# Madhudorai/encodec-pytorch

Hardware: AMD Instinct MI355X
Metric: audio-seconds/sec EnCodec24k train step, batch 32x1s (higher is better)
Workload: dtype f32; 1 GPU; config 3: 24 kHz mono full GAN (MS-STFT disc + Balancer); global_batch=32, parallelism=dp1

## Files before the change

### encodec-pytorch_amd/csrc/api.hip

```cpp
#include <stdarg.h>
#include <stdio.h>
#include <stdlib.h>
#include <string.h>

#include <atomic>
#include <mutex>

#include "common.h"
#include "prof.h"

namespace {
constexpr int kMaxSlots = 1 << 14;
struct ProfState {
    std::mutex mu;
    bool on = false;
    int next = 0;
    hipEvent_t ev0[kMaxSlots];
    hipEvent_t ev1[kMaxSlots];
    double flops[kMaxSlots];
    double bytes[kMaxSlots];
    bool timed[kMaxSlots];
    char tags[kMaxSlots][64];
    bool created = false;
};
ProfState g_prof;
std::atomic<bool> g_prof_on{false};

struct OptDef {
    EncxOpt id;
    const char* name;
    int64_t def;
};
constexpr OptDef kOpts[OPT_COUNT] = {
    {OPT_FFT, "FFT", 1}, {OPT_PW, "PW", 1}, {OPT_PW_TMAX, "PW_TMAX", 1024}, {OPT_PW_WG_TMAX, "PW_WG_TMAX", 12000}, {OPT_LSTM_FUSE, "LSTM_FUSE", 0},
    {OPT_LSTM_PERSIST, "LSTM_PERSIST", 1},
    {OPT_LSTM_WG_SPLITS, "LSTM_WG_SPLITS", 32},
    {OPT_FWR, "FWR", 256}, {OPT_DGR, "DGR", 256}, {OPT_WGR, "WGR", 2048},
    {OPT_WGR_WGS, "WGR_WGS", 256}, {OPT_FEAT_CODE, "FEAT_CODE", 1}, {OPT_CONV_CK, "CONV_CK", 64},
    {OPT_CONV_SPLIT, "CONV_SPLIT", 1024}, {OPT_CONV_WG_SPLIT, "CONV_WG_SPLIT", 1024},
    {OPT_CONV2, "CONV2", 7}, {OPT_CONV2_TILE, "CONV2_TILE", 0}, {OPT_CONV2_RED, "CONV2_RED", 64},
    {OPT_CONV2_KS, "CONV2_KS", 0}, {OPT_CONV2_WGS, "CONV2_WGS", 512},
    {OPT_CONV2_LOWT, "CONV2_LOWT", 0},
    {OPT_LSTM_SPIN, "LSTM_SPIN", 0}, {OPT_LSTM_FAULT, "LSTM_FAULT", 0},
    {OPT_BLAS, "BLAS", 3},
};
constexpr bool opts_in_order() {
    for (int i = 0; i < OPT_COUNT; ++i)
        if (kOpts[i].id != i) return false;
    return true;
}
static_assert(opts_in_order(), "kOpts must list every EncxOpt in enum order");
std::atomic<int64_t> g_opt[OPT_COUNT];
std::once_flag g_opt_once;
void opt_init() {
    std::call_once(g_opt_once, [] {
        for (int i = 0; i < OPT_COUNT; ++i) {
            char env[64];
            snprintf(env, sizeof(env), "ENCX_%s", kOpts[i].name);
            const char* v = getenv(env);
            g_opt[i].store(v ? atoll(v) : kOpts[i].def);
        }
    });
}
int opt_find(const char* name) {
    if (!name) return -1;
    if (!strncmp(name, "ENCX_", 5)) name += 5;
    for (int i = 0; i < OPT_COUNT; ++i)
        if (!strcmp(name, kOpts[i].name)) return i;
    return -1;
}
}

int64_t encx_opt(EncxOpt id) {
    opt_init();
    return g_opt[id].load(std::memory_order_relaxed);
}

// ... 119 lines not shown
```

### encodec-pytorch_amd/csrc/common.h

```cpp
#pragma once
#include <hip/hip_runtime.h>
#include <algorithm>
#include <stdint.h>

#include "../../include/encx.h"

#define ENCX_DEV __device__ __forceinline__

typedef float f32x16 __attribute__((ext_vector_type(16)));
typedef float f32x4 __attribute__((ext_vector_type(4)));
typedef float f32x2 __attribute__((ext_vector_type(2)));
typedef float f32x4u __attribute__((ext_vector_type(4), aligned(4)));
ENCX_DEV f32x4 ld4u(const float* p) { return *(const f32x4u*)p; }

#define ENCX_CHECK_LAUNCH()                                                    \
    do {                                                                       \
        hipError_t _e = hipGetLastError();                                     \
        if (_e != hipSuccess) return (int)_e;                                  \
    } while (0)
#define ENCX_REQUIRE(cond)                                                     \
    do {                                                                       \
        if (!(cond)) return ENCX_EINVAL;                                       \
    } while (0)

// ... 128 lines not shown
    t.x = id % gx;
    t.y = (id / gx) % gy;
    t.z = id / (gx * gy);
    return t;
}

static inline int64_t cdiv(int64_t a, int64_t b) { return (a + b - 1) / b; }

enum EncxOpt {
    OPT_FFT,
    OPT_PW,
    OPT_PW_TMAX,
    OPT_PW_WG_TMAX,
    OPT_LSTM_FUSE,
    OPT_LSTM_PERSIST,
    OPT_LSTM_WG_SPLITS,
    OPT_FWR,
    OPT_DGR,
    OPT_WGR,
    OPT_WGR_WGS,
    OPT_FEAT_CODE,
    OPT_CONV_CK,
    OPT_CONV_SPLIT,
    OPT_CONV_WG_SPLIT,
    OPT_CONV2,
    OPT_CONV2_TILE,
    OPT_CONV2_RED,
    OPT_CONV2_KS,
    OPT_CONV2_WGS,
    OPT_CONV2_LOWT,
    OPT_LSTM_SPIN,
    OPT_LSTM_FAULT,
    OPT_BLAS,
    OPT_COUNT
};
int64_t encx_opt(EncxOpt id);

int encx_sgemm(hipStream_t st, bool ta, bool tb, int m, int n, int k, const float* A, int lda, const float* B,
               int ldb, float* C, int ldc, bool accumulate, int batch = 1, int64_t sa = 0, int64_t sb = 0,
               int64_t sc = 0);
```

### encodec-pytorch_amd/csrc/gemm.h

```cpp
#pragma once
#include "common.h"

template <class EP, class = void>
struct ep_npre { static constexpr int value = 0; };
template <class EP>
struct ep_npre<EP, decltype((void)EP::NPRE)> { static constexpr int value = EP::NPRE; };

template <class LD, class = void>
struct ld_vec { static constexpr bool value = false; };
template <class LD>
struct ld_vec<LD, decltype((void)LD::VEC)> { static constexpr bool value = LD::VEC; };

template <int BM, int BN, int WM, int WN, int BK, class LD, class EP>
__global__ __launch_bounds__(256) void gemm_kernel(LD ld, EP ep, int M, int N, int Kred, int kchunk) {
    constexpr int TM = BM / WM / 32, TN = BN / WN / 32;
    __shared__ float As[BK][BM + 1];
    __shared__ float Bs[BK][BN + 1];
    const int tid = threadIdx.x, lane = tid & 63, wave = tid >> 6;
    const int wm0 = (wave / WN) * TM * 32, wn0 = (wave % WN) * TN * 32;
    const int m0 = blockIdx.y * BM, n0 = blockIdx.x * BN;
    const int kbeg = blockIdx.z * kchunk, kend = min(Kred, kbeg + kchunk);
    const int h = lane >> 5, l32 = lane & 31;
    f32x16 acc[TM][TN];
#pragma unroll
    for (int i = 0; i < TM; ++i)
#pragma unroll
        for (int j = 0; j < TN; ++j) acc[i][j] = (f32x16){0};
    constexpr int EA = BM * BK / 256, EB = BN * BK / 256;
    static_assert(EA * 256 == BM * BK && EB * 256 == BN * BK, "tile/thread mismatch");
    float ra[EA], rb[EB];
    constexpr bool VEC = ld_vec<LD>::value;
    static_assert(!VEC || (EA % 4 == 0 && EB % 4 == 0), "quad staging");
    auto quad_a = [&](int e, int& m, int& k) {
        const int i = tid + e * 256;
        if (LD::A_K_FAST) { m = i / (BK / 4); k = (i - m * (BK / 4)) * 4; }
        else { k = i / (BM / 4); m = (i - k * (BM / 4)) * 4; }
    };
    auto quad_b = [&](int e, int& k, int& n) {
        const int i = tid + e * 256;
        if (LD::B_N_FAST) { k = i / (BN / 4); n = (i - k * (BN / 4)) * 4; }
        else { n = i / (BK / 4); k = (i - n * (BK / 4)) * 4; }
    };
    auto fetch = [&](int k0) {
        if constexpr (VEC) {
#pragma unroll
            for (int e = 0; e < EA / 4; ++e) {
                int m, k;
                quad_a(e, m, k);
                const int gm = m0 + m, gk = k0 + k;
                const bool whole = LD::A_K_FAST ? (gm < M && gk + 3 < kend) : (gm + 3 < M && gk < kend);
                f32x4 v;
                if (whole) {
                    v = ld.a4(gm, gk);
                } else {
// ... 135 lines not shown
                for (int r = 0; r < 16; ++r) {
                    const int m = m0 + wm0 + i * 32 + mfma_row(r, lane);
                    if (m < M && n < N) ep(m, n, acc[i][j][r]);
                }
            }
        }
}

struct GemmShape {
    int BM, BN;
    int64_t blocks;
};

static inline GemmShape gemm_shape(int M, int N) {
    GemmShape s;
    if (N <= 48) { s.BM = 128; s.BN = 32; }
    else if (N <= 96) { s.BM = 128; s.BN = 64; }
    else if (cdiv(N, 128) * cdiv(M, 128) < 512) { s.BM = 64; s.BN = 64; }
    else { s.BM = 128; s.BN = 128; }
    s.blocks = cdiv(N, s.BN) * cdiv(M, s.BM);
    return s;
}

static inline int gemm_splits(int M, int N, int Kred, int min_k = 256, int max_splits = 32) {
    GemmShape s = gemm_shape(M, N);
    int sp = (int)cdiv(1024, s.blocks);
    int cap = Kred / min_k;
    if (sp > cap) sp = cap;
    if (sp > max_splits) sp = max_splits;
    return sp < 1 ? 1 : sp;
}

template <class LD, class EP>
int gemm_launch(const LD& ld, const EP& ep, int M, int N, int Kred, hipStream_t st, int splits = 1) {
    GemmShape s = gemm_shape(M, N);
    const int kchunk = splits > 1 ? (int)(cdiv(cdiv(Kred, splits), 32) * 32) : Kred;
    const int z = (int)cdiv(Kred, kchunk);
    if (s.BN == 32) {
        hipLaunchKernelGGL((gemm_kernel<128, 32, 4, 1, 32, LD, EP>), dim3(cdiv(N, 32), cdiv(M, 128), z),
                           dim3(256), 0, st, ld, ep, M, N, Kred, kchunk);
    } else if (s.BN == 64 && s.BM == 128) {
        hipLaunchKernelGGL((gemm_kernel<128, 64, 2, 2, 32, LD, EP>), dim3(cdiv(N, 64), cdiv(M, 128), z),
                           dim3(256), 0, st, ld, ep, M, N, Kred, kchunk);
    } else if (s.BN == 64) {
        hipLaunchKernelGGL((gemm_kernel<64, 64, 2, 2, 32, LD, EP>), dim3(cdiv(N, 64), cdiv(M, 64), z),
                           dim3(256), 0, st, ld, ep, M, N, Kred, kchunk);
    } else {
        hipLaunchKernelGGL((gemm_kernel<128, 128, 2, 2, 32, LD, EP>), dim3(cdiv(N, 128), cdiv(M, 128), z),
                           dim3(256), 0, st, ld, ep, M, N, Kred, kchunk);
    }
    ENCX_CHECK_LAUNCH();
    return 0;
}

static inline int gemm_splits_128(int M, int N, int Kred, int min_k = 256, int max_splits = 32) {
    const int blocks = (int)(cdiv(N, 128) * cdiv(M, 128));
    int sp = (int)cdiv(1024, blocks);
    const int cap = Kred / min_k;
    if (sp > cap) sp = cap;
    if (sp > max_splits) sp = max_splits;
    return sp < 1 ? 1 : sp;
}
template <class LD, class EP>
int gemm_launch_128(const LD& ld, const EP& ep, int M, int N, int Kred, hipStream_t st, int splits) {
    const int kchunk = splits > 1 ? (int)(cdiv(cdiv(Kred, splits), 32) * 32) : Kred;
    const int z = (int)cdiv(Kred, kchunk);
    hipLaunchKernelGGL((gemm_kernel<128, 128, 2, 2, 32, LD, EP>), dim3(cdiv(N, 128), cdiv(M, 128), z),
                       dim3(256), 0, st, ld, ep, M, N, Kred, kchunk);
    ENCX_CHECK_LAUNCH();
    return 0;
// ... 8 lines not shown
```

### encodec-pytorch_amd/csrc/rvq.hip

```cpp
#include "common.h"
#include "prof.h"
#include "gemm.h"

namespace {

constexpr int NT = 256;

struct Rows {
    const float* p;
    int64_t sB, sT, sD;
    int Tf;
    FastDiv fTf;
    ENCX_DEV float at(int n, int d) const {
        const int b = (int)fdiv((uint32_t)n, fTf), t = n - b * Tf;
        return p[b * sB + t * sT + d * sD];
    }
};

ENCX_DEV uint32_t ord_key(float f) {
    uint32_t u = __float_as_uint(f);
    return (u & 0x80000000u) ? ~u : (u | 0x80000000u);
}
ENCX_DEV uint64_t umin64(uint64_t a, uint64_t b) { return a < b ? a : b; }
ENCX_DEV uint64_t shfl_xor64(uint64_t v, int o) {
// ... 94 lines not shown
        ee[c] = v;
    }
    f32x16 acc[1];
    acc[0] = (f32x16){0};
    const float* ap = As + h * AR_ROWS + wm0 + l32;
    const float* bp = Bs + h * AR_BS + wn0 + l32;
#pragma unroll 4
    for (int dp = 0; dp < D; dp += 2) {
        const float av = ap[dp * AR_ROWS];
        acc[0] = mfma32(av, bp[dp * AR_BS], acc[0]);
    }
    __syncthreads();
#pragma unroll
    for (int r = 0; r < 16; ++r) {
        const int row = wm0 + mfma_row(r, lane);
        uint64_t best = ~0ull;
#pragma unroll
        for (int j = 0; j < 1; ++j) {
            const int c = wn0 + j * 32 + l32, k = k0 + c;
            if (k < Kc) {
                const float v = (xx[row] - 2.f * acc[j][r]) + ee[c];
                best = umin64(best, ((uint64_t)ord_key(v) << 32) | (uint32_t)k);
            }
        }
#pragma unroll
        for (int o = 16; o > 0; o >>= 1) best = umin64(best, shfl_xor64(best, o));
        if (l32 == 0) part[wave & 1][row] = best;
    }
    __syncthreads();
    if (tid < AR_ROWS && n0 + tid < N)
        atomicMin((unsigned long long*)&keys[n0 + tid], (unsigned long long)umin64(part[0][tid], part[1][tid]));
}

constexpr int DR_ROWS = 32;

__global__ __launch_bounds__(NT) void rvq_argmin_direct(Rows x, const float* embed, uint64_t* keys,
                                                        int N, int D, int Kc) {
    extern __shared__ float sm[];
    float* es = sm;
    float* xs = sm + NT * (D + 1);
    __shared__ uint64_t part[4];
    const int tid = threadIdx.x, lane = tid & 63, wave = tid >> 6;
    const int n0 = blockIdx.x * DR_ROWS, k = blockIdx.y * NT + tid;
    for (int i = tid; i < NT * D; i += NT) {
        int c = i / D, d = i - c * D, kk = blockIdx.y * NT + c;
        es[c * (D + 1) + d] = kk < Kc ? embed[(int64_t)kk * D + d] : 0.f;
    }
    for (int i = tid; i < DR_ROWS * D; i += NT) {
        int r = i / D, d = i - r * D;
        xs[i] = (n0 + r < N) ? x.at(n0 + r, d) : 0.f;
    }
    __syncthreads();
    for (int r = 0; r < DR_ROWS; ++r) {
        float s = 0.f;
        for (int d = 0; d < D; ++d) {
            float df = xs[r * D + d] - es[tid * (D + 1) + d];
            s = fmaf(df, df, s);
        }
        uint64_t key = k < Kc ? (((uint64_t)ord_key(s) << 32) | (uint32_t)k) : ~0ull;
#pragma unroll
        for (int o = 32; o > 0; o >>= 1) key = umin64(key, shfl_xor64(key, o));
        if (lane == 0) part[wave] = key;
        __syncthreads();
        if (tid == 0 && n0 + r < N) {
            uint64_t b = umin64(umin64(part[0], part[1]), umin64(part[2], part[3]));
            atomicMin((unsigned long long*)&keys[n0 + r], (unsigned long long)b);
// ... 21 lines not shown
    __shared__ float red[16];
    float s = 0.f;
    for (int64_t i = (int64_t)blockIdx.x * NT + threadIdx.x; i < total; i += (int64_t)gridDim.x * NT) {
        int64_t bd = i / Tf;
        int t = (int)(i - bd * Tf);
        int64_t b = bd / D;
        int d = (int)(bd - b * D);
        const int64_t k = idx[b * Tf + t];
        const float x = xin[i];
        const float q = embed[k * D + d];
        const float qs = ste ? x + (q - x) : q;
        res[i] = x - qs;
        if (out) out[i] = first ? qs : out[i] + qs;
        if (cdir) cdir[i] = first ? (x - qs) : cdir[i] + (x - qs);
        const float df = qs - x;
        s = fmaf(df, df, s);
    }
    s = block_sum(s, red);
    if (parts && threadIdx.x == 0) parts[blockIdx.x] = s;
}

__global__ void rvq_gather_kernel(const float* embed, const int64_t* idx, float* out, int D, int Tf,
                                  int64_t total, int acc) {
    int64_t i = (int64_t)blockIdx.x * blockDim.x + threadIdx.x;
    if (i >= total) return;
    int64_t bd = i / Tf;
    int t = (int)(i - bd * Tf);
    int64_t b = bd / D;
    int d = (int)(bd - b * D);
    float q = embed[idx[b * Tf + t] * D + d];
    out[i] = acc ? out[i] + q : q;
}

struct LdOneHot {
    static constexpr bool A_K_FAST = true, B_N_FAST = false;
    Rows x;
    const int64_t* idx;
    int D;
    ENCX_DEV float a(int c, int n) const { return idx[n] == c ? 1.f : 0.f; }
    ENCX_DEV float b(int n, int d) const { return d < D ? x.at(n, d) : 1.f; }
};
struct EpSlab {
    float* ws;
    int Kc, W;
    ENCX_DEV void operator()(int c, int d, float v) const {
        ws[((int64_t)blockIdx.z * Kc + c) * W + d] = v;
    }
};

template <int MODE>
__global__ void bucket_finish(const float* ws, int S, int Kc, int D, float* cs, float* ea,
                              float* means, int64_t* bins, float decay, float one_m) {
    const int c = blockIdx.x, W = D + 1;
    const float cnt = MODE == 1 ? sum_strided(ws + (int64_t)c * W + D, S, (int64_t)Kc * W) : 0.f;
    for (int d = threadIdx.x; d <= D; d += blockDim.x) {
        const float s = sum_strided(ws + (int64_t)c * W + d, S, (int64_t)Kc * W);
        if (MODE == 2) {
            means[(int64_t)c * W + d] = s;
        } else if (MODE == 0) {
            if (d < D) {
                float* p = ea + (int64_t)c * D + d;
                *p = fmaf(s, one_m, *p * decay);
            } else {
                cs[c] = fmaf(s, one_m, cs[c] * decay);
            }
        } else {
            if (d < D) {
                if (cnt > 0.f) means[(int64_t)c * D + d] = s / cnt;
            } else {
                bins[c] = (int64_t)cnt;
            }
        }
    }
}

template <int MODE>
int bucket_run(Rows x, const int64_t* idx, int N, int D, int Kc, float* ws, float* cs, float* ea,
               float* means, int64_t* bins, float decay, float one_m, hipStream_t st) {
    const int splits = gemm_splits(Kc, D + 1, N);
    const int S = gemm_slabs(N, splits);
    int rc = gemm_launch(LdOneHot{x, idx, D}, EpSlab{ws, Kc, D + 1}, Kc, D + 1, N, st, splits);
    if (rc) return rc;
    hipLaunchKernelGGL(bucket_finish<MODE>, dim3(Kc), dim3(D + 1 < 64 ? 64 : 256), 0, st, ws, S, Kc, D,
                       cs, ea, means, bins, decay, one_m);
    ENCX_CHECK_LAUNCH();
    return 0;
}

__global__ void ema_from_sums(const float* sums, int D, float* cs, float* ea, float decay, float one_m) {
    const int c = blockIdx.x, W = D + 1;
    for (int d = threadIdx.x; d <= D; d += blockDim.x) {
        const float s = sums[(int64_t)c * W + d];
        if (d < D) {
            float* p = ea + (int64_t)c * D + d;
            *p = fmaf(s, one_m, *p * decay);
        } else {
            cs[c] = fmaf(s, one_m, cs[c] * decay);
        }
    }
}

__global__ void ema_normalize(const float* cs, const float* ea, float* embed, int D, int Kc,
                              float eps, float keps) {
    __shared__ float red[16];
    float s = 0.f;
    for (int i = threadIdx.x; i < Kc; i += blockDim.x) s += cs[i];
    s = block_sum(s, red);
    const int c = blockIdx.x;
    const float sm = (cs[c] + eps) / (s + keps) * s;
    for (int d = threadIdx.x; d < D; d += blockDim.x)
        embed[(int64_t)c * D + d] = ea[(int64_t)c * D + d] / sm;
}

ENCX_DEV uint64_t splitmix(uint64_t z) {
    z += 0x9E3779B97F4A7C15ull;
    z = (z ^ (z >> 30)) * 0xBF58476D1CE4E5B9ull;
    z = (z ^ (z >> 27)) * 0x94D049BB133111EBull;
    return z ^ (z >> 31);
}

__global__ __launch_bounds__(NT) void sample_rows_kernel(const float* samples, float* out, int N,
                                                         int D, int num, uint64_t seed) {
    const int i = blockIdx.x * NT + threadIdx.x;
    if (num > N) {
        if (i >= num) return;
        int src = (int)(splitmix(seed ^ (0xA24BAED4963EE407ull * (uint64_t)(i + 1))) % (uint64_t)N);
        for (int d = 0; d < D; ++d) out[(int64_t)i * D + d] = samples[(int64_t)src * D + d];
        return;
    }
    if (i >= N) return;
    const uint64_t ki = splitmix(seed + (uint64_t)i);
    int rank = 0;
    for (int j = 0; j < N; ++j) {
        uint64_t kj = splitmix(seed + (uint64_t)j);
        rank += (kj < ki) || (kj == ki && j < i);
    }
    if (rank < num)
        for (int d = 0; d < D; ++d) out[(int64_t)rank * D + d] = samples[(int64_t)i * D + d];
}

Rows bdt_rows(const float* p, int64_t B, int64_t D, int64_t Tf) {
    Rows r;
    r.p = p; r.sB = D * Tf; r.sT = 1; r.sD = Tf; r.Tf = (int)Tf; r.fTf = make_fastdiv((uint32_t)Tf);
    return r;
// ... 81 lines not shown
    const float one_m = (float)(1.0 - (double)decay);
    int rc = bucket_run<0>(bdt_rows(x, B, D, Tf), idx, (int)(B * Tf), (int)D, (int)Kc, ws,
                           cluster_size, embed_avg, nullptr, nullptr, decay, one_m, st);
    if (rc) return rc;
    hipLaunchKernelGGL(ema_normalize, dim3(Kc), dim3(D < 64 ? 64 : (D > 256 ? 256 : D)), 0, st,
                       cluster_size, embed_avg, embed, (int)D, (int)Kc, eps,
                       (float)((double)Kc * (double)eps));
    ENCX_CHECK_LAUNCH();
    return 0;
}

int encx_rvq_code_sums(const float* x, const int64_t* idx, float* sums, float* ws, int64_t B,
                       int64_t D, int64_t Tf, int64_t Kc, encx_stream_t stream) {
    ENCX_REQUIRE(x && idx && sums && ws && B > 0 && D > 0 && D <= 256 && Tf > 0 && Kc > 0);
    return bucket_run<2>(bdt_rows(x, B, D, Tf), idx, (int)(B * Tf), (int)D, (int)Kc, ws, nullptr,
                         nullptr, sums, nullptr, 0.f, 0.f, (hipStream_t)stream);
}

int encx_rvq_ema_from_sums(const float* sums, float* cluster_size, float* embed_avg, float* embed,
                           int64_t D, int64_t Kc, float decay, float eps, encx_stream_t stream) {
    ENCX_REQUIRE(sums && cluster_size && embed_avg && embed && D > 0 && D <= 256 && Kc > 0);
    hipStream_t st = (hipStream_t)stream;
    const float one_m = (float)(1.0 - (double)decay);
    hipLaunchKernelGGL(ema_from_sums, dim3(Kc), dim3(D + 1 < 64 ? 64 : 256), 0, st, sums, (int)D,
                       cluster_size, embed_avg, decay, one_m);
    ENCX_CHECK_LAUNCH();
    hipLaunchKernelGGL(ema_normalize, dim3(Kc), dim3(D < 64 ? 64 : (D > 256 ? 256 : D)), 0, st,
                       cluster_size, embed_avg, embed, (int)D, (int)Kc, eps,
                       (float)((double)Kc * (double)eps));
    ENCX_CHECK_LAUNCH();
    return 0;
}

int encx_kmeans_step(const float* samples, float* means, int64_t* bins, int64_t* idx,
                     uint64_t* keys, float* ws, int64_t N, int64_t D, int64_t Kc,
                     encx_stream_t stream) {
    ENCX_REQUIRE(samples && means && bins && idx && keys && ws && N > 0 && D > 0 && D <= 256 && Kc > 0);
    hipStream_t st = (hipStream_t)stream;
    Rows r = nd_rows(samples, N, D);
    int rc = argmin_run(r, means, idx, keys, (int)N, (int)D, (int)Kc, 1, st);
    if (rc) return rc;
    return bucket_run<1>(r, idx, (int)N, (int)D, (int)Kc, ws, nullptr, nullptr, means, bins, 0.f,
                         0.f, st);
}

int encx_sample_rows(const float* samples, float* out, int64_t N, int64_t D, int64_t num,
                     uint64_t seed, encx_stream_t stream) {
    ENCX_REQUIRE(samples && out && N > 0 && D > 0 && num > 0);
    int64_t threads = num > N ? num : N;
    hipLaunchKernelGGL(sample_rows_kernel, dim3(cdiv(threads, NT)), dim3(NT), 0, (hipStream_t)stream,
                       samples, out, (int)N, (int)D, (int)num, seed);
    ENCX_CHECK_LAUNCH();
    return 0;
}

}
```

### encodec-pytorch_amd/encx/ops.py

```python
import contextlib
import ctypes
import os
import math
import operator

import numpy as np
import torch

from ._lib import (call, ptr, stream, lib, ensure_device, ENCX_PAD_ZERO, ENCX_PAD_REFLECT,
                   ENCX_ACT_NONE, ENCX_ACT_ELU)

ACT = {None: ENCX_ACT_NONE, 'none': ENCX_ACT_NONE, 'elu': ENCX_ACT_ELU}
PAD = {'reflect': ENCX_PAD_REFLECT, 'zero': ENCX_PAD_ZERO, 'constant': ENCX_PAD_ZERO}


def _f32(n, like):
    return torch.empty(int(n), device=like.device, dtype=torch.float32)


def _ws(nbytes, like):
    if nbytes == 0:
        return None
    return torch.empty((nbytes + 3) // 4, device=like.device, dtype=torch.float32)


def _check(x, name='x'):
    if not x.is_cuda or x.dtype != torch.float32:
        raise RuntimeError(f'encx: {name} must be a float32 tensor on the GPU '
                           f'(got {x.dtype} on {x.device}); the HIP path has no CPU fallback')
    ensure_device(x.device)


def extra_padding_for_conv1d(length, kernel_size, stride, padding_total=0):
    n_frames = (length - kernel_size + padding_total) / stride + 1
    ideal_length = (math.ceil(n_frames) - 1) * stride + (kernel_size - padding_total)
    return ideal_length - length


def conv_geometry(T, K, s, d, causal, pad_mode='reflect'):
    pt = (K - 1) * d - (s - 1)
    extra = extra_padding_for_conv1d(T, K, s, pt)
    if causal:
# ... 518 lines not shown
    B, D, T = res.shape
    N = B * T
    idx = torch.empty(N, device=res.device, dtype=torch.int64)
    keys = torch.empty(N, device=res.device, dtype=torch.int64)
    call('encx_rvq_argmin', ptr(res), ptr(embed), ptr(idx), ptr(keys), B, D, T, embed.shape[0],
         int(direct), stream())
    return idx


def kmeans(samples, num_clusters, num_iters, seed):
    N, D = samples.shape
    means = torch.empty(num_clusters, D, device=samples.device, dtype=torch.float32)
    call('encx_sample_rows', ptr(samples), ptr(means), N, D, num_clusters, seed & (2 ** 64 - 1), stream())
    bins = torch.zeros(num_clusters, device=samples.device, dtype=torch.int64)
    idx = torch.empty(N, device=samples.device, dtype=torch.int64)
    keys = torch.empty(N, device=samples.device, dtype=torch.int64)
    ws = _ws(lib.encx_rvq_bucket_workspace(N, D, num_clusters), samples)
    for _ in range(num_iters):
        call('encx_kmeans_step', ptr(samples), ptr(means), ptr(bins), ptr(idx), ptr(keys), ptr(ws),
             N, D, num_clusters, stream())
    return means, bins


def rvq_to_rows(res):
    B, D, T = res.shape
    out = torch.empty(B * T, D, device=res.device, dtype=torch.float32)
    call('encx_bdt_to_nd', ptr(res), ptr(out), B, D, T, stream())
    return out


_CB_DEFER = None


class CodebookSync:

    def __init__(self, sums, codebooks, decay, eps):
        self.sums, self.codebooks, self.decay, self.eps = sums, codebooks, decay, eps

    def apply(self):
        n_q, Kc, D1 = self.sums.shape
        for i, cb in enumerate(self.codebooks):
            call('encx_rvq_ema_from_sums', ptr(self.sums[i]), ptr(cb.cluster_size), ptr(cb.embed_avg),
                 ptr(cb.embed), D1 - 1, Kc, self.decay, self.eps, stream())


@contextlib.contextmanager
def defer_codebook_sync(pending: list):
    global _CB_DEFER
    prev, _CB_DEFER = _CB_DEFER, pending
    try:
        yield pending
    finally:
        _CB_DEFER = prev


class RVQTrainFn(torch.autograd.Function):

    @staticmethod
    def forward(ctx, emb, codebooks, decay, eps, sync=False, cw=1.0):
        _check(emb, 'emb')
        emb = emb.contiguous()
        B, D, T = emb.shape
        n_q = len(codebooks)
        numel = emb.numel()
        st = stream()
        res = [emb.clone(), torch.empty_like(emb)]
        out = torch.empty_like(emb)
        cdir = torch.empty_like(emb)
        P = lib.encx_rvq_apply_parts(B, D, T)
        parts = torch.empty(n_q, P, device=emb.device, dtype=torch.float32)
        commits = torch.empty(n_q, device=emb.device, dtype=torch.float32)
        codes = torch.empty(n_q, B * T, device=emb.device, dtype=torch.int64)
        keys = torch.empty(B * T, device=emb.device, dtype=torch.int64)
        Kc = codebooks[0].embed.shape[0]
        bws = _ws(lib.encx_rvq_bucket_workspace(B * T, D, Kc), emb)
        sums = None
        if sync and codebooks[0].training and torch.distributed.is_initialized() \
                and torch.distributed.get_world_size() > 1:
            sums = torch.empty(n_q, Kc, D + 1, device=emb.device, dtype=torch.float32)
        for i, cb in enumerate(codebooks):
            x = res[i % 2]
            cb.init_embed_(x)
            call('encx_rvq_argmin', ptr(x), ptr(cb.embed), ptr(codes[i]), ptr(keys), B, D, T,
                 cb.embed.shape[0], 0, st)
            call('encx_rvq_apply', ptr(x), ptr(res[(i + 1) % 2]), ptr(cb.embed), ptr(codes[i]),
                 ptr(out), ptr(cdir), ptr(parts[i]), B, D, T, int(i == 0), 1, st)
            if cb.training and sums is not None:
                call('encx_rvq_code_sums', ptr(x), ptr(codes[i]), ptr(sums[i]), ptr(bws), B, D, T, Kc, st)
            elif cb.training:
                call('encx_rvq_ema', ptr(x), ptr(codes[i]), ptr(cb.cluster_size), ptr(cb.embed_avg),
                     ptr(cb.embed), ptr(bws), B, D, T, cb.embed.shape[0], float(decay), float(eps), st)
            call('encx_reduce_sum', ptr(parts[i]), P, 1.0 / numel, ptr(commits[i:i + 1]), 0, st)
        if sums is not None:
            sync_ent = CodebookSync(sums, list(codebooks), float(decay), float(eps))
            if _CB_DEFER is not None:
                _CB_DEFER.append(sync_ent)
            else:
                torch.distributed.all_reduce(sums)
                sync_ent.apply()
        penalty = torch.empty(1, device=emb.device, dtype=torch.float32)
        call('encx_reduce_sum', ptr(commits), n_q, float(cw) / n_q, ptr(penalty), 0, st)
        ctx.save_for_backward(cdir)
        ctx.n_q, ctx.numel, ctx.cw = n_q, numel, float(cw)
        ctx.mark_non_differentiable(codes)
        return out, codes.view(n_q, B, T), penalty.view(())

    @staticmethod
    def backward(ctx, dq, dcodes, dpen):
        cdir, = ctx.saved_tensors
        n_q, numel = ctx.n_q, ctx.numel
        if dq is None:
            dq = torch.zeros_like(cdir)
        dq = dq.contiguous()
        demb = torch.empty_like(cdir)
        if dpen is None:
            call('encx_lincomb', ptr(dq), ptr(cdir), ptr(demb), demb.numel(), float(n_q), None, 0.0,
                 stream())
        else:
            call('encx_lincomb', ptr(dq), ptr(cdir), ptr(demb), demb.numel(), float(n_q),
                 ptr(dpen.contiguous().view(1)), 2.0 * ctx.cw / (n_q * numel), stream())
        return demb, None, None, None, None, None


def rvq_encode(emb, embeds):
    _check(emb, 'emb')
    emb = emb.contiguous()
    B, D, T = emb.shape
    res = emb.clone()
    codes = torch.empty(len(embeds), B * T, device=emb.device, dtype=torch.int64)
    keys = torch.empty(B * T, device=emb.device, dtype=torch.int64)
    for i, E in enumerate(embeds):
        call('encx_rvq_argmin', ptr(res), ptr(E), ptr(codes[i]), ptr(keys), B, D, T, E.shape[0], 0,
             stream())
        call('encx_rvq_apply', ptr(res), ptr(res), ptr(E), ptr(codes[i]), None, None, None, B, D, T,
             0, 0, stream())
    return codes.view(len(embeds), B, T)


def rvq_decode(codes, embeds):
    n_q, B, T = codes.shape
    D = embeds[0].shape[1]
    out = torch.empty(B, D, T, device=codes.device, dtype=torch.float32)
    codes = codes.contiguous()
    for i in range(n_q):
        call('encx_rvq_gather', ptr(embeds[i]), ptr(codes[i]), ptr(out), B, D, T, int(i > 0), stream())
    return out


class LSTMFn(torch.autograd.Function):

    @staticmethod
    def forward(ctx, x, skip, *weights):
        _check(x)
        x = x.contiguous()
        B, H, T = x.shape
        L = len(weights) // 4
        if B > LSTM_MAX_BATCH or H % 16 or H > 1024:
            raise NotImplementedError('encx LSTM: hidden % 16 == 0 and <= 1024 (lstm() splits the batch)')
        st = stream()
        wcat = _f32(L * 8 * H * H, x)
        wcatT = _f32(L * 8 * H * H, x)
        bsum = _f32(L * 4 * H, x)
        for l in range(L):
            w_ih, w_hh, b_ih, b_hh = (w.contiguous() for w in weights[4 * l:4 * l + 4])
            call('encx_lstm_pack', ptr(w_ih), ptr(w_hh), ptr(b_ih), ptr(b_hh), ptr(wcat), ptr(wcatT),
                 ptr(bsum), H, l, st)
        xt = _f32(B * T * H, x)
        Y = _f32(L * B * T * H, x)
        Cs = _f32(L * B * T * H, x)
        Gs = _f32(L * B * T * 4 * H, x)
        out = torch.empty_like(x)
        call('encx_lstm_fwd', ptr(x), ptr(wcat), ptr(bsum), ptr(xt), ptr(Y), ptr(Cs), ptr(Gs), ptr(out),
             int(bool(skip)), B, T, H, L, st)
        ctx.save_for_backward(xt, Y, Cs, Gs, wcatT)
        ctx.weights = weights
        ctx.skip = skip
# ... 546 lines not shown
```

### include/encx.h

```cpp
#ifndef ENCX_H
#define ENCX_H

#include <stddef.h>
#include <stdint.h>

#ifdef __cplusplus
extern "C" {
#endif

typedef struct ihipStream_t* encx_stream_t;

#define ENCX_OK 0
#define ENCX_EINVAL 9001

#define ENCX_PAD_ZERO 0
#define ENCX_PAD_REFLECT 1
#define ENCX_ACT_NONE 0
#define ENCX_ACT_ELU 1

int encx_version(void);
const char* encx_build_id(void);
const char* encx_strerror(int code);
int encx_option_count(void);
const char* encx_option_name(int i);
// ... 80 lines not shown
                      const float* ws, float* dx, float* dw1, float* db1, float* dw2, float* db2, float* dws,
                      float* dbs, int acc_w, int acc_b, float* wsp, int64_t B, int64_t C, int64_t T,
                      encx_stream_t stream);

size_t encx_channel_sum_workspace(int64_t C);
int encx_channel_sum(const float* dy, float* db, float* ws, int64_t B, int64_t C, int64_t T,
                     int accumulate, encx_stream_t stream);
int encx_normalize_fwd(const float* x, float* xn, float* scale, int64_t B, int64_t C, int64_t T,
                       encx_stream_t stream);
int encx_scale_rows(const float* x, const float* scale, float* y, int64_t B, int64_t CT,
                    encx_stream_t stream);
int encx_axpby(const float* x, float* y, int64_t n, float alpha, const float* alpha_dev,
               float beta, encx_stream_t stream);
int encx_l1_loss(const float* x, const float* y, float* loss, float* grad, float* ws, int64_t n,
                 encx_stream_t stream);

int encx_rvq_argmin(const float* res, const float* embed, int64_t* idx, uint64_t* keys,
                    int64_t B, int64_t D, int64_t Tf, int64_t Kc, int direct,
                    encx_stream_t stream);
int encx_rvq_apply(const float* x, float* res_out, const float* embed, const int64_t* idx,
                   float* out, float* commit_dir, float* commit_part, int64_t B, int64_t D,
                   int64_t Tf, int first, int ste, encx_stream_t stream);
int encx_rvq_gather(const float* embed, const int64_t* idx, float* out, int64_t B, int64_t D,
                    int64_t Tf, int accumulate, encx_stream_t stream);
int64_t encx_rvq_apply_parts(int64_t B, int64_t D, int64_t Tf);
size_t encx_rvq_bucket_workspace(int64_t N, int64_t D, int64_t Kc);
int encx_rvq_ema(const float* x, const int64_t* idx, float* cluster_size, float* embed_avg,
                 float* embed, float* ws, int64_t B, int64_t D, int64_t Tf, int64_t Kc,
                 float decay, float eps, encx_stream_t stream);
int encx_rvq_code_sums(const float* x, const int64_t* idx, float* sums, float* ws, int64_t B,
                       int64_t D, int64_t Tf, int64_t Kc, encx_stream_t stream);
int encx_rvq_ema_from_sums(const float* sums, float* cluster_size, float* embed_avg, float* embed,
                           int64_t D, int64_t Kc, float decay, float eps, encx_stream_t stream);
int encx_kmeans_step(const float* samples, float* means, int64_t* bins, int64_t* idx,
                     uint64_t* keys, float* ws, int64_t N, int64_t D, int64_t Kc,
                     encx_stream_t stream);
int encx_sample_rows(const float* samples, float* out, int64_t N, int64_t D, int64_t num,
                     uint64_t seed, encx_stream_t stream);
int encx_bdt_to_nd(const float* res, float* out, int64_t B, int64_t D, int64_t Tf,
                   encx_stream_t stream);
int encx_reduce_sum(const float* parts, int64_t n, float scale, float* out, int accumulate,
                    encx_stream_t stream);

size_t encx_mel_tables_floats(int64_t n_fft, int64_t n_mels);
int encx_spec_tables_window(float* tables, const float* window, int64_t n_fft, encx_stream_t stream);
int encx_mel_tables_init(float* tables, const float* mel_basis, int64_t n_fft, int64_t n_mels,
                         encx_stream_t stream);
size_t encx_mel_workspace_floats(int64_t B, int64_t T, int64_t n_fft, int64_t n_mels);
int encx_mel_loss(const float* x, const float* y, const float* tables, float* ws, float* loss,
                  float* grad, int64_t B, int64_t T, int64_t n_fft, int64_t n_mels,
                  encx_stream_t stream);

size_t encx_mel_loss_multi_workspace_floats(int64_t B, int64_t T, const int64_t* n_ffts, int64_t nscales);
int encx_mel_loss_multi(const float* x, const float* y, const float* const* tables, const int64_t* n_ffts,
                        int64_t nscales, float* ws, float* loss, float* grad, int64_t B, int64_t T,
                        encx_stream_t stream);
int encx_mel_logmel(const float* x, const float* tables, float* ws, float* out, int64_t B,
                    int64_t T, int64_t n_fft, int64_t n_mels, encx_stream_t stream);
int64_t encx_mel_frames(int64_t T, int64_t n_fft);
size_t encx_mel_logmel_framed_workspace_floats(int64_t B, int64_t T, int64_t n_fft, int64_t hop);
int encx_mel_logmel_framed(const float* x, const float* win_tables, const float* mel_basis, float* ws, float* out,
                           int64_t B, int64_t T, int64_t n_fft, int64_t hop, int64_t n_mels, encx_stream_t stream);

int encx_lincomb(const float* x, const float* z, float* out, int64_t n, float a, const float* bdev,
                 float bscale, encx_stream_t stream);
size_t encx_item_norm_workspace(int64_t B);
// ... 189 lines not shown
```

Measured before the change: 956.4 audio-seconds/sec.

## Batch RVQ codebook EMA, commit reduction and gather across quantizer layers

Keeps every layer's residual in one stacked buffer so the codebook EMA update for all quantizer layers runs as one batched one-hot GEMM plus batched finish and normalize kernels, instead of several launches per layer. The per-layer commit-loss reductions become one row-reduction kernel, and decoding sums all layers' codebook lookups in a single gather kernel. This cuts kernel launches and host call overhead in the RVQ stage. In exchange it uses more memory for the n_q+1 residual buffers and an n_q-times larger workspace, and the EMA update now runs after all argmins rather than between layers.

```diff
diff --git a/encodec-pytorch_amd/csrc/api.hip b/encodec-pytorch_amd/csrc/api.hip
--- a/encodec-pytorch_amd/csrc/api.hip
+++ b/encodec-pytorch_amd/csrc/api.hip
@@ -42,7 +42,7 @@
     {OPT_CONV2_KS, "CONV2_KS", 0}, {OPT_CONV2_WGS, "CONV2_WGS", 512},
     {OPT_CONV2_LOWT, "CONV2_LOWT", 0},
     {OPT_LSTM_SPIN, "LSTM_SPIN", 0}, {OPT_LSTM_FAULT, "LSTM_FAULT", 0},
-    {OPT_BLAS, "BLAS", 3},
+    {OPT_BLAS, "BLAS", 3}, {OPT_RVQ_BATCH, "RVQ_BATCH", 1},
 };
 constexpr bool opts_in_order() {
     for (int i = 0; i < OPT_COUNT; ++i)
diff --git a/encodec-pytorch_amd/csrc/common.h b/encodec-pytorch_amd/csrc/common.h
--- a/encodec-pytorch_amd/csrc/common.h
+++ b/encodec-pytorch_amd/csrc/common.h
@@ -184,6 +184,7 @@
     OPT_LSTM_SPIN,
     OPT_LSTM_FAULT,
     OPT_BLAS,
+    OPT_RVQ_BATCH,
     OPT_COUNT
 };
 int64_t encx_opt(EncxOpt id);
diff --git a/encodec-pytorch_amd/csrc/gemm.h b/encodec-pytorch_amd/csrc/gemm.h
--- a/encodec-pytorch_amd/csrc/gemm.h
+++ b/encodec-pytorch_amd/csrc/gemm.h
@@ -10,6 +10,15 @@
 struct ld_vec { static constexpr bool value = false; };
 template <class LD>
 struct ld_vec<LD, decltype((void)LD::VEC)> { static constexpr bool value = LD::VEC; };
+
+template <class LD, class = void>
+struct ld_kslab {
+    static __device__ __forceinline__ int z(const LD&) { return blockIdx.z; }
+};
+template <class LD>
+struct ld_kslab<LD, decltype((void)LD::BATCHED)> {
+    static __device__ __forceinline__ int z(const LD& ld) { return blockIdx.z % ld.S; }
+};
 
 template <int BM, int BN, int WM, int WN, int BK, class LD, class EP>
 __global__ __launch_bounds__(256) void gemm_kernel(LD ld, EP ep, int M, int N, int Kred, int kchunk) {
@@ -19,7 +28,7 @@
     const int tid = threadIdx.x, lane = tid & 63, wave = tid >> 6;
     const int wm0 = (wave / WN) * TM * 32, wn0 = (wave % WN) * TN * 32;
     const int m0 = blockIdx.y * BM, n0 = blockIdx.x * BN;
-    const int kbeg = blockIdx.z * kchunk, kend = min(Kred, kbeg + kchunk);
+    const int kbeg = ld_kslab<LD>::z(ld) * kchunk, kend = min(Kred, kbeg + kchunk);
     const int h = lane >> 5, l32 = lane & 31;
     f32x16 acc[TM][TN];
 #pragma unroll
@@ -221,10 +230,11 @@
 }
 
 template <class LD, class EP>
-int gemm_launch(const LD& ld, const EP& ep, int M, int N, int Kred, hipStream_t st, int splits = 1) {
+int gemm_launch(const LD& ld, const EP& ep, int M, int N, int Kred, hipStream_t st, int splits = 1,
+                int batch = 1) {
     GemmShape s = gemm_shape(M, N);
     const int kchunk = splits > 1 ? (int)(cdiv(cdiv(Kred, splits), 32) * 32) : Kred;
-    const int z = (int)cdiv(Kred, kchunk);
+    const int z = (int)cdiv(Kred, kchunk) * batch;
     if (s.BN == 32) {
         hipLaunchKernelGGL((gemm_kernel<128, 32, 4, 1, 32, LD, EP>), dim3(cdiv(N, 32), cdiv(M, 128), z),
                            dim3(256), 0, st, ld, ep, M, N, Kred, kchunk);
diff --git a/encodec-pytorch_amd/csrc/rvq.hip b/encodec-pytorch_amd/csrc/rvq.hip
--- a/encodec-pytorch_amd/csrc/rvq.hip
+++ b/encodec-pytorch_amd/csrc/rvq.hip
@@ -150,6 +150,8 @@
         atomicMin((unsigned long long*)&keys[n0 + tid], (unsigned long long)umin64(part[0][tid], part[1][tid]));
 }
 
+constexpr int RVQ_MAXQ = 32;
+
 constexpr int DR_ROWS = 32;
 
 __global__ __launch_bounds__(NT) void rvq_argmin_direct(Rows x, const float* embed, uint64_t* keys,
@@ -237,6 +239,35 @@
     out[i] = acc ? out[i] + q : q;
 }
 
+struct GatherArgs {
+    const int64_t* idx;
+    float* out;
+    int D, Tf, n_q;
+    int64_t total, N;
+    const float* embed[RVQ_MAXQ];
+};
+__global__ void rvq_gather_batch_kernel(GatherArgs a) {
+    int64_t i = (int64_t)blockIdx.x * blockDim.x + threadIdx.x;
+    if (i >= a.total) return;
+    int64_t bd = i / a.Tf;
+    int t = (int)(i - bd * a.Tf);
+    int64_t b = bd / a.D;
+    int d = (int)(bd - b * a.D);
+    const int64_t n = b * a.Tf + t;
+    float s = a.embed[0][a.idx[n] * a.D + d];
+    for (int l = 1; l < a.n_q; ++l) s = s + a.embed[l][a.idx[l * a.N + n] * a.D + d];
+    a.out[i] = s;
+}
+
+__global__ __launch_bounds__(NT) void reduce_rows_kernel(const float* parts, int64_t n, float scale, float* out) {
+    __shared__ float red[16];
+    const float* p = parts + (int64_t)blockIdx.x * n;
+    float s = 0.f;
+    for (int64_t i = threadIdx.x; i < n; i += NT) s += p[i];
+    s = block_sum(s, red);
+    if (threadIdx.x == 0) out[blockIdx.x] = s * scale;
+}
+
 struct LdOneHot {
     static constexpr bool A_K_FAST = true, B_N_FAST = false;
     Rows x;
@@ -253,9 +284,29 @@
     }
 };
 
+struct LdOneHotB {
+    static constexpr bool A_K_FAST = true, B_N_FAST = false;
+    static constexpr bool BATCHED = true;
+    Rows x;
+    const int64_t* idx;
+    int D, S;
+    int64_t xstride, istride;
+    ENCX_DEV float a(int c, int n) const { return idx[(blockIdx.z / S) * istride + n] == c ? 1.f : 0.f; }
+    ENCX_DEV float b(int n, int d) const {
+        if (d >= D) return 1.f;
+        const int bb = (int)fdiv((uint32_t)n, x.fTf), t = n - bb * x.Tf;
+        return x.p[(blockIdx.z / S) * xstride + bb * x.sB + t * x.sT + d * x.sD];
+    }
+};
+struct LayerBufs {
+    float* cs[RVQ_MAXQ];
+    float* ea[RVQ_MAXQ];
+    float* embed[RVQ_MAXQ];
+};
+
 template <int MODE>
-__global__ void bucket_finish(const float* ws, int S, int Kc, int D, float* cs, float* ea,
-                              float* means, int64_t* bins, float decay, float one_m) {
+ENCX_DEV void bucket_finish_body(const float* ws, int S, int Kc, int D, float* cs, float* ea,
+                                 float* means, int64_t* bins, float decay, float one_m) {
     const int c = blockIdx.x, W = D + 1;
     const float cnt = MODE == 1 ? sum_strided(ws + (int64_t)c * W + D, S, (int64_t)Kc * W) : 0.f;
     for (int d = threadIdx.x; d <= D; d += blockDim.x) {
@@ -280,6 +331,20 @@
 }
 
 template <int MODE>
+__global__ void bucket_finish(const float* ws, int S, int Kc, int D, float* cs, float* ea,
+                              float* means, int64_t* bins, float decay, float one_m) {
+    bucket_finish_body<MODE>(ws, S, Kc, D, cs, ea, means, bins, decay, one_m);
+}
+template <int MODE>
+__global__ void bucket_finish_batch(const float* ws, int S, int Kc, int D, LayerBufs L, float* sums,
+                                    float decay, float one_m) {
+    const int l = blockIdx.y;
+    bucket_finish_body<MODE>(ws + (int64_t)l * S * Kc * (D + 1), S, Kc, D, MODE == 0 ? L.cs[l] : nullptr,
+                             MODE == 0 ? L.ea[l] : nullptr,
+                             MODE == 2 ? sums + (int64_t)l * Kc * (D + 1) : nullptr, nullptr, decay, one_m);
+}
+
+template <int MODE>
 int bucket_run(Rows x, const int64_t* idx, int N, int D, int Kc, float* ws, float* cs, float* ea,
                float* means, int64_t* bins, float decay, float one_m, hipStream_t st) {
     const int splits = gemm_splits(Kc, D + 1, N);
@@ -292,7 +357,7 @@
     return 0;
 }
 
-__global__ void ema_from_sums(const float* sums, int D, float* cs, float* ea, float decay, float one_m) {
+ENCX_DEV void ema_from_sums_body(const float* sums, int D, float* cs, float* ea, float decay, float one_m) {
     const int c = blockIdx.x, W = D + 1;
     for (int d = threadIdx.x; d <= D; d += blockDim.x) {
         const float s = sums[(int64_t)c * W + d];
@@ -305,9 +370,16 @@
     }
 }
 
-__global__ void ema_normalize(const float* cs, const float* ea, float* embed, int D, int Kc,
-                              float eps, float keps) {
-    __shared__ float red[16];
+__global__ void ema_from_sums(const float* sums, int D, float* cs, float* ea, float decay, float one_m) {
+    ema_from_sums_body(sums, D, cs, ea, decay, one_m);
+}
+__global__ void ema_from_sums_batch(const float* sums, int D, int Kc, LayerBufs L, float decay, float one_m) {
+    const int l = blockIdx.y;
+    ema_from_sums_body(sums + (int64_t)l * Kc * (D + 1), D, L.cs[l], L.ea[l], decay, one_m);
+}
+
+ENCX_DEV void ema_normalize_body(const float* cs, const float* ea, float* embed, int D, int Kc,
+                                 float eps, float keps, float* red) {
     float s = 0.f;
     for (int i = threadIdx.x; i < Kc; i += blockDim.x) s += cs[i];
     s = block_sum(s, red);
@@ -315,6 +387,16 @@
     const float sm = (cs[c] + eps) / (s + keps) * s;
     for (int d = threadIdx.x; d < D; d += blockDim.x)
         embed[(int64_t)c * D + d] = ea[(int64_t)c * D + d] / sm;
+}
+__global__ void ema_normalize(const float* cs, const float* ea, float* embed, int D, int Kc,
+                              float eps, float keps) {
+    __shared__ float red[16];
+    ema_normalize_body(cs, ea, embed, D, Kc, eps, keps, red);
+}
+__global__ void ema_normalize_batch(LayerBufs L, int D, int Kc, float eps, float keps) {
+    __shared__ float red[16];
+    const int l = blockIdx.y;
+    ema_normalize_body(L.cs[l], L.ea[l], L.embed[l], D, Kc, eps, keps, red);
 }
 
 ENCX_DEV uint64_t splitmix(uint64_t z) {
@@ -462,6 +544,120 @@
     return 0;
 }
 
+namespace {
+int fill_bufs(LayerBufs& L, float* const* cs, float* const* ea, float* const* embed, int64_t n_q) {
+    for (int i = 0; i < RVQ_MAXQ; ++i) {
+        const bool on = i < n_q;
+        if (on && !(cs[i] && ea[i] && (!embed || embed[i]))) return ENCX_EINVAL;
+        L.cs[i] = on ? cs[i] : nullptr;
+        L.ea[i] = on ? ea[i] : nullptr;
+        L.embed[i] = on && embed ? embed[i] : nullptr;
+    }
+    return 0;
+}
+int sums_batch_run(const float* xs, const int64_t* codes, float* ws, int64_t B, int64_t D, int64_t Tf,
+                   int64_t Kc, int64_t n_q, int* S, hipStream_t st) {
+    const int N = (int)(B * Tf);
+    const int splits = gemm_splits((int)Kc, (int)D + 1, N);
+    *S = gemm_slabs(N, splits);
+    LdOneHotB ld{bdt_rows(xs, B, D, Tf), codes, (int)D, *S, B * D * Tf, B * Tf};
+    return gemm_launch(ld, EpSlab{ws, (int)Kc, (int)D + 1}, (int)Kc, (int)D + 1, N, st, splits, (int)n_q);
+}
+void normalize_batch_run(const LayerBufs& L, int64_t D, int64_t Kc, int64_t n_q, float eps, hipStream_t st) {
+    hipLaunchKernelGGL(ema_normalize_batch, dim3(Kc, n_q), dim3(D < 64 ? 64 : (D > 256 ? 256 : D)), 0, st,
+                       L, (int)D, (int)Kc, eps, (float)((double)Kc * (double)eps));
+}
+}
+
+size_t encx_rvq_ema_batch_workspace(int64_t N, int64_t D, int64_t Kc, int64_t n_q) {
+    if (!encx_opt(OPT_RVQ_BATCH) || n_q <= 0 || n_q > RVQ_MAXQ) return 0;
+    return (size_t)n_q * encx_rvq_bucket_workspace(N, D, Kc);
+}
+
+int encx_rvq_ema_batch(const float* xs, const int64_t* codes, float* const* cluster_size,
+                       float* const* embed_avg, float* const* embed, float* ws, int64_t B, int64_t D,
+                       int64_t Tf, int64_t Kc, int64_t n_q, float decay, float eps,
+                       encx_stream_t stream) {
+    ENCX_REQUIRE(xs && codes && cluster_size && embed_avg && embed && ws && B > 0 && D > 0 && D <= 256 &&
+                 Tf > 0 && Kc > 0 && n_q > 0 && n_q <= RVQ_MAXQ);
+    LayerBufs L;
+    int rc = fill_bufs(L, cluster_size, embed_avg, embed, n_q);
+    if (rc) return rc;
+    encx_prof_scope ps((hipStream_t)stream, n_q * (2.0 * B * Tf * Kc * (D + 1)),
+                       n_q * (4.0 * (B * D * Tf + 4 * Kc * D) + 8.0 * B * Tf), "rvq_ema_batch");
+    hipStream_t st = (hipStream_t)stream;
+    const float one_m = (float)(1.0 - (double)decay);
+    int S;
+    rc = sums_batch_run(xs, codes, ws, B, D, Tf, Kc, n_q, &S, st);
+    if (rc) return rc;
+    hipLaunchKernelGGL(bucket_finish_batch<0>, dim3(Kc, n_q), dim3(D + 1 < 64 ? 64 : 256), 0, st, ws, S,
+                       (int)Kc, (int)D, L, nullptr, decay, one_m);
+    ENCX_CHECK_LAUNCH();
+    normalize_batch_run(L, D, Kc, n_q, eps, st);
+    ENCX_CHECK_LAUNCH();
+    return 0;
+}
+
+int encx_rvq_code_sums_batch(const float* xs, const int64_t* codes, float* sums, float* ws, int64_t B,
+                             int64_t D, int64_t Tf, int64_t Kc, int64_t n_q, encx_stream_t stream) {
+    ENCX_REQUIRE(xs && codes && sums && ws && B > 0 && D > 0 && D <= 256 && Tf > 0 && Kc > 0 && n_q > 0 &&
+                 n_q <= RVQ_MAXQ);
+    hipStream_t st = (hipStream_t)stream;
+    int S;
+    int rc = sums_batch_run(xs, codes, ws, B, D, Tf, Kc, n_q, &S, st);
+    if (rc) return rc;
+    LayerBufs L = {};
+    hipLaunchKernelGGL(bucket_finish_batch<2>, dim3(Kc, n_q), dim3(D + 1 < 64 ? 64 : 256), 0, st, ws, S,
+                       (int)Kc, (int)D, L, sums, 0.f, 0.f);
+    ENCX_CHECK_LAUNCH();
+    return 0;
+}
+
+int encx_rvq_ema_from_sums_batch(const float* sums, float* const* cluster_size, float* const* embed_avg,
+                                 float* const* embed, int64_t D, int64_t Kc, int64_t n_q, float decay,
+                                 float eps, encx_stream_t stream) {
+    ENCX_REQUIRE(sums && cluster_size && embed_avg && embed && D > 0 && D <= 256 && Kc > 0 && n_q > 0 &&
+                 n_q <= RVQ_MAXQ);
+    LayerBufs L;
+    int rc = fill_bufs(L, cluster_size, embed_avg, embed, n_q);
+    if (rc) return rc;
+    hipStream_t st = (hipStream_t)stream;
+    const float one_m = (float)(1.0 - (double)decay);
+    hipLaunchKernelGGL(ema_from_sums_batch, dim3(Kc, n_q), dim3(D + 1 < 64 ? 64 : 256), 0, st, sums, (int)D,
+                       (int)Kc, L, decay, one_m);
+    ENCX_CHECK_LAUNCH();
+    normalize_batch_run(L, D, Kc, n_q, eps, st);
+    ENCX_CHECK_LAUNCH();
+    return 0;
+}
+
+int encx_rvq_commit_reduce(const float* parts, float* commits, float* penalty, int64_t n_parts, int64_t n_q,
+                           float commit_scale, float penalty_scale, encx_stream_t stream) {
+    ENCX_REQUIRE(parts && commits && penalty && n_parts > 0 && n_q > 0);
+    hipStream_t st = (hipStream_t)stream;
+    hipLaunchKernelGGL(reduce_rows_kernel, dim3(n_q), dim3(NT), 0, st, parts, n_parts, commit_scale, commits);
+    ENCX_CHECK_LAUNCH();
+    hipLaunchKernelGGL(reduce_rows_kernel, dim3(1), dim3(NT), 0, st, commits, n_q, penalty_scale, penalty);
+    ENCX_CHECK_LAUNCH();
+    return 0;
+}
+
+int encx_rvq_gather_batch(const float* const* embeds, const int64_t* idx, float* out, int64_t B, int64_t D,
+                          int64_t Tf, int64_t n_q, encx_stream_t stream) {
+    ENCX_REQUIRE(embeds && idx && out && B > 0 && D > 0 && Tf > 0 && n_q > 0 && n_q <= RVQ_MAXQ);
+    GatherArgs a;
+    a.idx = idx; a.out = out; a.D = (int)D; a.Tf = (int)Tf; a.n_q = (int)n_q;
+    a.total = B * D * Tf; a.N = B * Tf;
+    for (int i = 0; i < RVQ_MAXQ; ++i) {
+        a.embed[i] = i < n_q ? embeds[i] : nullptr;
+        ENCX_REQUIRE(i >= n_q || embeds[i]);
+    }
+    encx_prof_scope ps((hipStream_t)stream, 0.0, 4.0 * B * D * Tf * (2 + 3 * (n_q - 1)), "rvq_gather_batch", false);
+    hipLaunchKernelGGL(rvq_gather_batch_kernel, dim3(cdiv(a.total, 256)), dim3(256), 0, (hipStream_t)stream, a);
+    ENCX_CHECK_LAUNCH();
+    return 0;
+}
+
 int encx_kmeans_step(const float* samples, float* means, int64_t* bins, int64_t* idx,
                      uint64_t* keys, float* ws, int64_t N, int64_t D, int64_t Kc,
                      encx_stream_t stream) {
diff --git a/encodec-pytorch_amd/encx/ops.py b/encodec-pytorch_amd/encx/ops.py
--- a/encodec-pytorch_amd/encx/ops.py
+++ b/encodec-pytorch_amd/encx/ops.py
@@ -7,7 +7,7 @@
 import numpy as np
 import torch
 
-from ._lib import (call, ptr, stream, lib, ensure_device, ENCX_PAD_ZERO, ENCX_PAD_REFLECT,
+from ._lib import (call, ptr, stream, lib, ensure_device, get_option, ENCX_PAD_ZERO, ENCX_PAD_REFLECT,
                    ENCX_ACT_NONE, ENCX_ACT_ELU)
 
 ACT = {None: ENCX_ACT_NONE, 'none': ENCX_ACT_NONE, 'elu': ENCX_ACT_ELU}
@@ -592,6 +592,16 @@
 _CB_DEFER = None
 
 
+def _ptrs(tensors):
+    return (ctypes.c_void_p * len(tensors))(*[ptr(t) for t in tensors])
+
+
+def _rvq_batch(embeds):
+    if 'ENCX_LIB' in os.environ and not hasattr(lib.load(), 'encx_rvq_ema_batch'):
+        return False
+    return bool(get_option('RVQ_BATCH')) and len(embeds) <= 32 and all(E.shape == embeds[0].shape for E in embeds)
+
+
 class CodebookSync:
 
     def __init__(self, sums, codebooks, decay, eps):
@@ -599,6 +609,12 @@
 
     def apply(self):
         n_q, Kc, D1 = self.sums.shape
+        cbs = self.codebooks
+        if _rvq_batch([cb.embed for cb in cbs]):
+            call('encx_rvq_ema_from_sums_batch', ptr(self.sums), _ptrs([cb.cluster_size for cb in cbs]),
+                 _ptrs([cb.embed_avg for cb in cbs]), _ptrs([cb.embed for cb in cbs]), D1 - 1, Kc, n_q,
+                 self.decay, self.eps, stream())
+            return
         for i, cb in enumerate(self.codebooks):
             call('encx_rvq_ema_from_sums', ptr(self.sums[i]), ptr(cb.cluster_size), ptr(cb.embed_avg),
                  ptr(cb.embed), D1 - 1, Kc, self.decay, self.eps, stream())
@@ -624,7 +640,13 @@
         n_q = len(codebooks)
         numel = emb.numel()
         st = stream()
-        res = [emb.clone(), torch.empty_like(emb)]
+        batch = _rvq_batch([cb.embed for cb in codebooks]) and len({bool(cb.training) for cb in codebooks}) == 1
+        if batch:
+            xs = torch.empty(n_q + 1, B, D, T, device=emb.device, dtype=torch.float32)
+            xs[0].copy_(emb)
+            res = list(xs.unbind(0))
+        else:
+            res = [emb.clone(), torch.empty_like(emb)]
         out = torch.empty_like(emb)
         cdir = torch.empty_like(emb)
         P = lib.encx_rvq_apply_parts(B, D, T)
@@ -633,24 +655,33 @@
         codes = torch.empty(n_q, B * T, device=emb.device, dtype=torch.int64)
         keys = torch.empty(B * T, device=emb.device, dtype=torch.int64)
         Kc = codebooks[0].embed.shape[0]
-        bws = _ws(lib.encx_rvq_bucket_workspace(B * T, D, Kc), emb)
+        bws = _ws(lib.encx_rvq_ema_batch_workspace(B * T, D, Kc, n_q) if batch else
+                  lib.encx_rvq_bucket_workspace(B * T, D, Kc), emb)
         sums = None
         if sync and codebooks[0].training and torch.distributed.is_initialized() \
                 and torch.distributed.get_world_size() > 1:
             sums = torch.empty(n_q, Kc, D + 1, device=emb.device, dtype=torch.float32)
         for i, cb in enumerate(codebooks):
-            x = res[i % 2]
+            x = res[i] if batch else res[i % 2]
             cb.init_embed_(x)
             call('encx_rvq_argmin', ptr(x), ptr(cb.embed), ptr(codes[i]), ptr(keys), B, D, T,
                  cb.embed.shape[0], 0, st)
-            call('encx_rvq_apply', ptr(x), ptr(res[(i + 1) % 2]), ptr(cb.embed), ptr(codes[i]),
-                 ptr(out), ptr(cdir), ptr(parts[i]), B, D, T, int(i == 0), 1, st)
+            call('encx_rvq_apply', ptr(x), ptr(res[i + 1] if batch else res[(i + 1) % 2]), ptr(cb.embed),
+                 ptr(codes[i]), ptr(out), ptr(cdir), ptr(parts[i]), B, D, T, int(i == 0), 1, st)
+            if batch:
+                continue
             if cb.training and sums is not None:
                 call('encx_rvq_code_sums', ptr(x), ptr(codes[i]), ptr(sums[i]), ptr(bws), B, D, T, Kc, st)
             elif cb.training:
                 call('encx_rvq_ema', ptr(x), ptr(codes[i]), ptr(cb.cluster_size), ptr(cb.embed_avg),
                      ptr(cb.embed), ptr(bws), B, D, T, cb.embed.shape[0], float(decay), float(eps), st)
             call('encx_reduce_sum', ptr(parts[i]), P, 1.0 / numel, ptr(commits[i:i + 1]), 0, st)
+        if batch and codebooks[0].training and sums is not None:
+            call('encx_rvq_code_sums_batch', ptr(xs), ptr(codes), ptr(sums), ptr(bws), B, D, T, Kc, n_q, st)
+        elif batch and codebooks[0].training:
+            call('encx_rvq_ema_batch', ptr(xs), ptr(codes), _ptrs([cb.cluster_size for cb in codebooks]),
+                 _ptrs([cb.embed_avg for cb in codebooks]), _ptrs([cb.embed for cb in codebooks]), ptr(bws),
+                 B, D, T, Kc, n_q, float(decay), float(eps), st)
         if sums is not None:
             sync_ent = CodebookSync(sums, list(codebooks), float(decay), float(eps))
             if _CB_DEFER is not None:
@@ -659,7 +690,11 @@
                 torch.distributed.all_reduce(sums)
                 sync_ent.apply()
         penalty = torch.empty(1, device=emb.device, dtype=torch.float32)
-        call('encx_reduce_sum', ptr(commits), n_q, float(cw) / n_q, ptr(penalty), 0, st)
+        if batch:
+            call('encx_rvq_commit_reduce', ptr(parts), ptr(commits), ptr(penalty), P, n_q, 1.0 / numel,
+                 float(cw) / n_q, st)
+        else:
+            call('encx_reduce_sum', ptr(commits), n_q, float(cw) / n_q, ptr(penalty), 0, st)
         ctx.save_for_backward(cdir)
         ctx.n_q, ctx.numel, ctx.cw = n_q, numel, float(cw)
         ctx.mark_non_differentiable(codes)
@@ -702,6 +737,9 @@
     D = embeds[0].shape[1]
     out = torch.empty(B, D, T, device=codes.device, dtype=torch.float32)
     codes = codes.contiguous()
+    if _rvq_batch(embeds[:n_q]):
+        call('encx_rvq_gather_batch', _ptrs(embeds[:n_q]), ptr(codes), ptr(out), B, D, T, n_q, stream())
+        return out
     for i in range(n_q):
         call('encx_rvq_gather', ptr(embeds[i]), ptr(codes[i]), ptr(out), B, D, T, int(i > 0), stream())
     return out
diff --git a/include/encx.h b/include/encx.h
--- a/include/encx.h
+++ b/include/encx.h
@@ -136,6 +136,20 @@
                        int64_t D, int64_t Tf, int64_t Kc, encx_stream_t stream);
 int encx_rvq_ema_from_sums(const float* sums, float* cluster_size, float* embed_avg, float* embed,
                            int64_t D, int64_t Kc, float decay, float eps, encx_stream_t stream);
+size_t encx_rvq_ema_batch_workspace(int64_t N, int64_t D, int64_t Kc, int64_t n_q);
+int encx_rvq_ema_batch(const float* xs, const int64_t* codes, float* const* cluster_size,
+                       float* const* embed_avg, float* const* embed, float* ws, int64_t B, int64_t D,
+                       int64_t Tf, int64_t Kc, int64_t n_q, float decay, float eps,
+                       encx_stream_t stream);
+int encx_rvq_code_sums_batch(const float* xs, const int64_t* codes, float* sums, float* ws, int64_t B,
+                             int64_t D, int64_t Tf, int64_t Kc, int64_t n_q, encx_stream_t stream);
+int encx_rvq_ema_from_sums_batch(const float* sums, float* const* cluster_size, float* const* embed_avg,
+                                 float* const* embed, int64_t D, int64_t Kc, int64_t n_q, float decay,
+                                 float eps, encx_stream_t stream);
+int encx_rvq_commit_reduce(const float* parts, float* commits, float* penalty, int64_t n_parts, int64_t n_q,
+                           float commit_scale, float penalty_scale, encx_stream_t stream);
+int encx_rvq_gather_batch(const float* const* embeds, const int64_t* idx, float* out, int64_t B, int64_t D,
+                          int64_t Tf, int64_t n_q, encx_stream_t stream);
 int encx_kmeans_step(const float* samples, float* means, int64_t* bins, int64_t* idx,
                      uint64_t* keys, float* ws, int64_t N, int64_t D, int64_t Kc,
                      encx_stream_t stream);
```

New measurement: 962.4 audio-seconds/sec (median of 6 runs). No clear change (+0.6%).
